# felixchenfy/Monocular-Visual-Odometry

Hardware: AMD Instinct MI355X
Metric: frames/sec (extract+match+5-kf BA), 640x480 / 2000 kp, 1->8 MI355X (higher is better)
Workload: dtype u8 (extract/match) + f64 (BA); 1 GPU

## Files before the change

include/mvo_hip.h:

```cpp
#ifndef MVO_HIP_H
#define MVO_HIP_H
#include <stdint.h>

#ifdef __cplusplus
extern "C" {
#endif

#define MVO_OK 0
#define MVO_ERR_INVALID (-1)
#define MVO_ERR_NO_DEVICE (-2)
#define MVO_ERR_CAPACITY (-3)
#define MVO_ERR_HIP (-4)
#define MVO_ERR_STATE (-5)

typedef struct mvo_ctx mvo_ctx;

typedef struct {
    float x, y, size, angle, response;
    int32_t octave, class_id;
} mvo_keypoint;

typedef struct {
    int32_t queryIdx, trainIdx, imgIdx;
    float distance;
// ... 272 lines not shown
                                  double* angles);
int mvo_rodrigues(const double* rvec, double* R);
int mvo_invert_pose(const double* T, double* T_inv);

int mvo_ba_launch_stats(int device, long long* launches, long long* windows, double* ms, int reset);
int mvo_debug_ba_service_times(int device, double* out5);
int mvo_debug_ba_resident_stats(int device, long long* windows, long long* grid_starts);
int mvo_debug_ba_resident_cycles(int device, double* shader_cycles);
int mvo_debug_ba_path_switches(int device, long long* n);
int mvo_debug_ba_demand_replay(const double* times, int n, uint8_t* decisions);
int mvo_profile_enable(mvo_ctx* ctx, int on);
int mvo_profile_reset(mvo_ctx* ctx);
typedef struct {
    char name[48];
    int64_t launches;
    double total_ms;
} mvo_kernel_time;
int mvo_profile_get(mvo_ctx* ctx, mvo_kernel_time* out, int cap);

int mvo_debug_set(const char* key, int value);
int mvo_debug_ba_trace_enable(mvo_ctx* ctx, int on);
int mvo_debug_get_ba_trace(mvo_ctx* ctx, mvo_ba_handle* handle, double* rows, int cap, int* n);
int mvo_debug_get_ba_plan(mvo_ctx* ctx, mvo_ba_handle* handle, int* wgs, int* nsplit, int32_t* wg_pt_start, int cap);
int mvo_debug_get_ba_phases(mvo_ctx* ctx, long long* cycles, int n, int* wgs);
int mvo_debug_get_level(mvo_ctx* ctx, int level, int blurred, uint8_t* out, int cap, int* w, int* h, int* stride);
int mvo_debug_get_candidates(mvo_ctx* ctx, void* out, int cap, int* n);
int mvo_debug_get_undistort_map(mvo_ctx* ctx, int32_t* ix, int32_t* iy, uint8_t* ax, uint8_t* ay, int cap);

int mvo_debug_get_pnp(mvo_ctx* ctx, double* models, int32_t* counts, int cap, int32_t* info);

int mvo_debug_get_essential(mvo_ctx* ctx, int32_t* counts, int cap_iters, int32_t* info);

int mvo_debug_get_homography(mvo_ctx* ctx, int32_t* counts, int cap_iters, int32_t* info);

int mvo_debug_get_recover_pose(mvo_ctx* ctx, int32_t* good, int32_t* chosen, double* R1R2t, uint8_t* masks, int cap);
int mvo_debug_get_homography_decomposition(mvo_ctx* ctx, double* Hn, double* w, int32_t* branch, double* Rs,
                                           double* ts, double* normals, int32_t* rejected);
int mvo_debug_get_init_finish(mvo_ctx* ctx, float* p_curr, double* cosang, double* pixdist, int cap, int* n);

#ifdef __cplusplus
}
#endif
#endif
```

monocular-visual-odometry_amd/__init__.py:

```python
import ctypes as C
import os

import numpy as np

from . import synth

_HERE = os.path.dirname(os.path.abspath(__file__))
LIB_PATH = os.path.join(_HERE, "csrc", "libmvo_hip.so")
HEADER_PATH = os.path.join(os.path.dirname(_HERE), "include", "mvo_hip.h")

MVO_OK, MVO_ERR_INVALID, MVO_ERR_NO_DEVICE, MVO_ERR_CAPACITY, MVO_ERR_HIP, MVO_ERR_STATE = 0, -1, -2, -3, -4, -5

KEYPOINT_DTYPE = np.dtype([("x", "<f4"), ("y", "<f4"), ("size", "<f4"), ("angle", "<f4"),
                           ("response", "<f4"), ("octave", "<i4"), ("class_id", "<i4")])
DMATCH_DTYPE = np.dtype([("queryIdx", "<i4"), ("trainIdx", "<i4"), ("imgIdx", "<i4"), ("distance", "<f4")])
CANDIDATE_DTYPE = np.dtype([("x", "<i2"), ("y", "<i2"), ("level_score", "<i4"), ("harris", "<f4"), ("angle", "<f4")])
DISTRIBUTE_CANDIDATE_DTYPE = np.dtype([("x", "<i4"), ("y", "<i4"), ("level", "<i4"), ("score", "<i4")])


class OrbParams(C.Structure):
    _fields_ = [("nfeatures", C.c_int32), ("scale_factor", C.c_float), ("nlevels", C.c_int32),
                ("fast_threshold", C.c_int32), ("max_keypoints", C.c_int32), ("grid_size", C.c_int32),
                ("grid_max_per_cell", C.c_int32), ("pyramid_interpolation", C.c_int32)]

# ... 634 lines not shown
        sts = (BaStats * len(problems))()
        self._chk(self.lib.mvo_ba_solve_batch(self.h, prs, len(problems), sts))
        return [(k["poses"].reshape(-1, 4, 4), k["points"], {f: getattr(sts[i], f) for f, _ in BaStats._fields_})
                for i, k in enumerate(keeps)]

    def ba_set_mode(self, mode):
        self._chk(self.lib.mvo_ba_set_mode(self.h, {"latency": 0, "throughput": 1, "shared": 2}[mode]))

    def ba_trace_enable(self, on=True):
        self._chk(self.lib.mvo_debug_ba_trace_enable(self.h, int(on)))

    def ba_trace(self, handle=None, raw_rows=0):
        out = np.zeros((512, 4))
        n = C.c_int()
        self._chk(self.lib.mvo_debug_get_ba_trace(self.h, handle[0] if handle else None, _p(out),
                                                  -int(raw_rows) if raw_rows else 512, C.byref(n)))
        return out[:n.value].copy()

    def ba_plan(self, handle=None):
        g, ns = C.c_int(), C.c_int()
        pt = np.zeros(257, np.int32)
        self._chk(self.lib.mvo_debug_get_ba_plan(self.h, handle[0] if handle else None, C.byref(g), C.byref(ns), _p(pt), 257))
        return dict(wgs=g.value, nsplit=ns.value & 0xffff, groups=max(1, ns.value >> 16), wg_pt_start=pt[:g.value + 1].copy())

    def map_create(self):
        m = C.c_void_p()
        self._chk(self.lib.mvo_map_create(self.h, C.byref(m)))
        return m

    def map_release(self, m):
        self.lib.mvo_map_release.restype = None
        self.lib.mvo_map_release(self.h, m)

    def map_upload(self, m, pos, desc):
        pos = np.ascontiguousarray(pos, np.float32).reshape(-1, 3)
        desc = np.ascontiguousarray(desc, np.uint8).reshape(-1, 32)
        assert len(pos) == len(desc)
        self._chk(self.lib.mvo_map_upload(self.h, m, _p(pos), _p(desc), len(pos)))

    def map_update_positions(self, m, pos, first=0):
        pos = np.ascontiguousarray(pos, np.float32).reshape(-1, 3)
        self._chk(self.lib.mvo_map_update_positions(self.h, m, _p(pos), int(first), len(pos)))

    def map_points_in_view(self, m, T_w_c, K, cols, rows, cap):
        T = np.ascontiguousarray(T_w_c, np.float64).reshape(4, 4)
        idx = np.zeros(max(cap, 1), np.int32)
# ... 445 lines not shown
```

monocular-visual-odometry_amd/csrc/ba_host.cpp:

```cpp
#include <algorithm>
#include <atomic>
#include <cmath>
#include <cstdio>
#include <condition_variable>
#include <cstdlib>
#include <cstring>
#include <chrono>
#include <deque>
#include <map>
#include <mutex>
#include <thread>
#include <vector>

#include "ba_types.h"
#include "mvo_internal.h"

int ba_kernel_set_lds_limit();
hipError_t ba_kernel_launch(const BaBatch& batch, int max_wgs, size_t lds_bytes, hipStream_t stream, int profile, int nr, int slots);
int ba_solver_class(int n);
hipError_t ba_service_launch(const BaServiceArgs& a, hipStream_t stream);

void ba_service_free(int device, void* p, bool host);

int g_ba_use_mfma = 1;
// ... 784 lines not shown
                if (plan_trace)
                    std::fprintf(stderr, "[mvo plan] G %d rows_in_lds %d chunks %d pieces %d pt_passes %d maxEg %d maxLg %d uarea %zu B lds %zu B (budget %d) %s\n",
                                 G, all_lds, nseq, npar, P.npt, maxEg, maxLg, uarea * 8, P.lds, BA_LDS_BUDGET, fits ? "fits" : "-");
                if (all_lds && g_ba_edge_rows != 0) {
                    if (uarea < (size_t)BA_MSTRIDE * (maxEg + 2 * F)) fits = false;
                    break;
                }
            }
        }
        if (fits && maxEg <= BA_EDGE_SLOTS * BA_THREADS && maxLg < 32000) break;
        if (G >= BA_MAX_WGS)
            return mvo_set_err(ctx, MVO_ERR_CAPACITY, "BA window too large for the LDS-resident solver", hipSuccess);
        {
            int next = BA_MAX_WGS;
            for (int c : {2, 4, 8, 16, 32, 64, 128, 256, per_xcd / 2, per_xcd, 2 * per_xcd, 4 * per_xcd, 8 * per_xcd})
                if (c > G && c < next) next = c;
            G = next;
        }
    }
    g_stage_times.lap(0);
    P.nsplit = nsplit;
    P.npar = npar;
    P.nseq = nseq;
    P.uarea = uarea;
    P.G = G;
    P.maxEg = maxEg;
    P.maxLg = maxLg;
    P.groups = 1;
    if (G > 32 && g_ba_groups) {
        int K = 2;
        while (G / K > 32 && K < 8) K *= 2;
        if (G % K == 0 && G / K <= 32 && uarea >= (size_t)K * (size_t)(nlow + nhp)) P.groups = K;
    }
    P.slice = (nlow + G / P.groups - 1) / (G / P.groups);
    std::vector<int>&e_pose = SC.e_pose, &e_point = SC.e_point, &ptstart = SC.ptstart, &ptlist = SC.ptlist;
    std::vector<double>& e_uv = SC.e_uv;
    e_pose.resize(E);
    e_point.resize(E);
    ptstart.assign(L + 1, 0);
    ptlist.resize(E);
    e_uv.resize(2 * (size_t)E);
    {
        std::vector<int>& cur = SC.cur;
        cur.resize((size_t)G * std::max(F, 1));
        for (int g = 0; g < G; ++g)
            for (int q = 0; q < F; ++q) cur[(size_t)g * F + q] = wg_pose[(size_t)g * (F + 1) + q];
        for (int e : act) {
            const int k = cur[(size_t)owner[p->edge_point[e]] * F + p->edge_pose[e]]++;
            e_pose[k] = p->edge_pose[e];
            e_point[k] = p->edge_point[e];
            e_uv[2 * (size_t)k] = p->edge_uv[2 * (size_t)e];
            e_uv[2 * (size_t)k + 1] = p->edge_uv[2 * (size_t)e + 1];
        }
    }
    for (int k = 0; k < E; ++k) ptstart[e_point[k] + 1]++;
// ... 366 lines not shown
    if (H->launched) service_wait(service_for(ctx ? ctx->device : H->ws.device), &H->job, 1);
    ws_free(H->ws);
    delete H;
}

int ba_get_trace(mvo_ctx* ctx, mvo_ba_handle* H, double* rows, int cap, int* n) {
    BaWorkspace* ws = H ? &H->ws : (ctx->ba_pool && !ctx->ba_pool->ws.empty() ? ctx->ba_pool->ws[0] : nullptr);
    if (!ws || !ws->pin) return mvo_set_err(ctx, MVO_ERR_STATE, "no bundle adjustment has run", hipSuccess);
    const BaStatsDev* s = (const BaStatsDev*)(ws->pin + ws->plan.m_stats);
    const int m = cap < 0 ? std::min(-cap, BA_TRACE_MAX) : std::min(std::min(s->trials, BA_TRACE_MAX), cap);
    if (rows) std::memcpy(rows, ws->pin + ws->plan.m_trace, (size_t)m * sizeof(BaTraceRow));
    if (n) *n = m;
    return MVO_OK;
}
int ba_get_plan(mvo_ctx* ctx, mvo_ba_handle* H, int* G, int* nsplit, int32_t* wg_pt, int cap) {
    BaWorkspace* ws = H ? &H->ws : (ctx->ba_pool && !ctx->ba_pool->ws.empty() ? ctx->ba_pool->ws[0] : nullptr);
    if (!ws) return mvo_set_err(ctx, MVO_ERR_STATE, "no bundle adjustment has been planned", hipSuccess);
    if (G) *G = ws->plan.G;
    if (nsplit) *nsplit = ws->plan.nsplit | (ws->plan.groups > 1 ? ws->plan.groups << 16 : 0);
    if (wg_pt)
        for (int i = 0; i <= ws->plan.G && i < cap; ++i) wg_pt[i] = ws->plan.wg_pt[i];
    return MVO_OK;
}
void ba_service_times(int device, double* out5) {
    for (int i = 0; i < 5; ++i) out5[i] = 0;
    if (device < 0 || device >= 16) return;
    BaService* sp;
    {
        std::lock_guard<std::mutex> lk(*g_service_start);
        sp = g_service[device & 15];
    }
    if (!sp) return;
    std::lock_guard<std::mutex> lk(sp->m);
    out5[0] = sp->t_idle, out5[1] = sp->t_batch, out5[2] = sp->t_launch, out5[3] = sp->t_sync, out5[4] = sp->t_post;
}
void ba_service_park(int device) {
    if (device < 0 || device >= 16) return;
    BaService* sp;
    {
        std::lock_guard<std::mutex> lk(*g_service_start);
        sp = g_service[device & 15];
    }
    if (!sp) return;
    std::unique_lock<std::mutex> lk(sp->m);
    if (!sp->resident) return;
    sp->park_requested = true;
// ... 53 lines not shown
```

monocular-visual-odometry_amd/csrc/ba_kernels.hip:

```cpp
#include "ba_types.h"
#include "mvo_internal.h"

typedef ba_u64 u64;
#ifndef MVO_KERNEL_SIM
typedef __attribute__((address_space(1))) double gdouble;
typedef __attribute__((address_space(1))) const u64 gcu64;
typedef __attribute__((address_space(1))) u64 gu64;
#define BA_AS_GLOBAL_D(p) ((gdouble*)(p))
#define BA_AS_GLOBAL_CU64(p) ((gcu64*)(p))
#define BA_AS_GLOBAL_U64(p) ((gu64*)(p))
#else
typedef double gdouble;
typedef const u64 gcu64;
typedef u64 gu64;
#define BA_AS_GLOBAL_D(p) (p)
#define BA_AS_GLOBAL_CU64(p) (p)
#define BA_AS_GLOBAL_U64(p) (p)
#endif

#define PH_BEGIN() long long ph_t = PROF ? (long long)__builtin_amdgcn_s_memtime() : 0
#define PH_END(id)                                                       \
    do {                                                                 \
        if (PROF) {                                                      \
            long long ph_n = (long long)__builtin_amdgcn_s_memtime();    \
// ... 789 lines not shown
    const int msteps = (ncol + 3) / 4;
    const int msplit = (msteps + B.nsplit - 1) / B.nsplit;
    const int chunk_cols = 4 * npar * msplit;
    const short* pkt_g = B.pk_of_tile;
    int pk4[4] = {-1, -1, -1, -1};
    if (do_schur && wave < B.npair * npar) {
#pragma unroll
        for (int j = 0; j < 4; ++j) pk4[j] = pkt_g[(wave % B.npair) * 256 + ((lane >> 4) + 4 * j) * 16 + (lane & 15)];
    }
    EdgeRegs er;
#pragma unroll
    for (int c = 0; c < 6; ++c) er.a0[c] = er.a1[c] = er.x[c] = 0;
    const bool have0 = SLOTS > 0 && tid < Eg, have1 = SLOTS > 1 && tid + BA_THREADS < Eg;
    const int e0_p = have0 ? W.epose[tid] : 0, e0_l = have0 ? W.ept[tid] : 0, e0_sl = have0 ? sSlot[e0_p] : -1;
    constexpr int nslot = SLOTS;
    constexpr int e2_first = SLOTS == 0 ? 0 : BA_THREADS;
#define BA_EDGE_FROM_LDS(BODY, el_)                                          \
    do {                                                                     \
        EdgeRegs r1_;                                                        \
        double ee_[2];                                                       \
        const double* q_ = W.E2 + BA_E2S * ((el_)-e2_first);                 \
        _Pragma("unroll") for (int c_ = 0; c_ < 6; ++c_) {                   \
            r1_.a0[c_] = q_[c_];                                             \
            r1_.a1[c_] = q_[6 + c_];                                         \
            r1_.x[c_] = q_[12 + c_];                                         \
        }                                                                    \
        ee_[0] = q_[18];                                                     \
        ee_[1] = q_[19];                                                     \
        const int p1_ = W.epose[el_];                                        \
        (void)p1_;                                                           \
        BODY(el_, r1_, W.ept[el_], sSlot[p1_], ee_)                          \
    } while (0);
#define BA_EDGES(BODY)                                                       \
    if (nslot > 0 && have0) do { BODY(tid, er, e0_l, e0_sl, ee0) } while (0); \
    if (nslot > 1 && have1) BA_EDGE_FROM_LDS(BODY, tid + BA_THREADS)         \
    if (nslot == 0)                                                          \
        for (int el0_ = tid; el0_ < Eg; el0_ += BA_THREADS) BA_EDGE_FROM_LDS(BODY, el0_)

    int hp_npass = 1;
    {
        const int mcap = (int)(B.uarea / BA_MSTRIDE);
        for (;; ++hp_npass) {
            int tot = 0;
            for (int p = 0; p < B.F; ++p) {
                const int n_p = sPoseStart[p + 1] - sPoseStart[p];
                tot += min(n_p, ((n_p + hp_npass - 1) / hp_npass + 1) & ~1);
            }
            if (tot <= mcap) break;
            if (hp_npass > Eg) {
                error = 1;
                break;
            }
        }
    }
    const bool hp_tables = hp_npass <= BA_HP_PASSES;
    auto hp_slice_row = [&](int q, int row) {
        if (tid < B.F) {
            int off = 0, lo = 0, hi = 0;
            for (int pp = 0; pp <= tid; ++pp) {
                const int s0 = sPoseStart[pp], n_p = sPoseStart[pp + 1] - s0;
                const int h = ((n_p + hp_npass - 1) / hp_npass + 1) & ~1;
                off += hi - lo;
                lo = min(s0 + q * h, s0 + n_p);
                hi = min(s0 + (q + 1) * h, s0 + n_p);
            }
            sSlc[0][row][tid] = (short)lo;
            sSlc[1][row][tid] = (short)hi;
            sSlc[2][row][tid] = (short)off;
        }
    };
    if (hp_tables && !error)
        for (int q = 0; q < hp_npass; ++q) hp_slice_row(q, q);
    int nfp = 0, hp_pa0 = -1, hp_pb0 = -1, hp_pa1 = -1, hp_pb1 = -1;
    for (int p = 0; p < B.F; ++p) {
        if (sSlot[p] < 0) continue;
        if (nfp == 2 * wave) hp_pa0 = p;
        if (nfp == 2 * wave + 1) hp_pb0 = p;
        if (nfp == 2 * (wave + BA_WAVES)) hp_pa1 = p;
        if (nfp == 2 * (wave + BA_WAVES) + 1) hp_pb1 = p;
        ++nfp;
    }
    __syncthreads();

    int piv_hoff = 0;
    if (NR == 32 && n > 0) {
        const int lsh = NR == 32 ? 4 : (n <= 32 ? 4 : (n <= 64 ? 3 : 2)), LPR = 1 << lsh, jj = tid & (LPR - 1);
        const int qi = min(tid >> lsh, n - 1), q0 = min(jj, n - 1), q1 = min(jj + LPR, n - 1);
        piv_hoff = (36 * sSlotPose[qi / 6] + 7 * (qi % 6)) | (36 * sSlotPose[q0 / 6] + 7 * (q0 % 6)) << 10 | (36 * sSlotPose[q1 / 6] + 7 * (q1 % 6)) << 20;
    }
    for (it = 0; any_free && !error && it < B.max_it; ++it) {
        PH_BEGIN();
// ... 10 lines not shown
            const double J0[6] = {x * y / z2 * f, -(1 + (x * x / z2)) * f, y / z * f, -1. / z * f, 0, x / z2 * f};   \
            const double J1[6] = {(1 + y * y / z2) * f, -x * y / z2 * f, -x / z * f, 0, -1. / z * f, y / z2 * f};    \
            _Pragma("unroll") for (int c = 0; c < 6; ++c) {                                                         \
                r.a0[c] = sw * (B.lc00 * J0[c] + B.lc01 * J1[c]);                                                   \
                r.a1[c] = sw * (B.lc11 * J1[c]);                                                                    \
            }                                                                                                       \
        } else {                                                                                                    \
            _Pragma("unroll") for (int c = 0; c < 6; ++c) r.a0[c] = r.a1[c] = 0;                                    \
        }                                                                                                           \
        ee[0] = sw * ew[0];                                                                                         \
        ee[1] = sw * ew[1];                                                                                         \
        _Pragma("unroll") for (int c = 0; c < 6; ++c) r.x[c] = 0;                                                   \
        if (!B.fix_points) {                                                                                        \
            const double* R = sR + 9 * (p);                                                                         \
            const double t0[3] = {f, 0, -x / z * f}, t1[3] = {0, f, -y / z * f};                                    \
            _Pragma("unroll") for (int c = 0; c < 3; ++c) {                                                         \
                double j0 = -1. / z * (t0[0] * R[c] + t0[1] * R[3 + c] + t0[2] * R[6 + c]);                         \
                double j1 = -1. / z * (t1[0] * R[c] + t1[1] * R[3 + c] + t1[2] * R[6 + c]);                         \
                r.x[c] = sw * (B.lc00 * j0 + B.lc01 * j1);                                                          \
                r.x[3 + c] = sw * (B.lc11 * j1);                                                                    \
            }                                                                                                       \
        }                                                                                                           \
    }
        if (nslot > 0 && have0) BA_LINEARIZE(tid, er, e0_p, e0_sl, ee0)
        for (int el = nslot == 0 ? tid : tid + BA_THREADS; nslot != 1 && el < Eg; el += BA_THREADS) {
            EdgeRegs r1;
            double ee[2];
            const int p1 = W.epose[el], sl1 = sSlot[p1];
            BA_LINEARIZE(el, r1, p1, sl1, ee)
            double* q = W.E2 + BA_E2S * (el - e2_first);
#pragma unroll
            for (int c = 0; c < 6; ++c) {
                q[c] = r1.a0[c];
                q[6 + c] = r1.a1[c];
                q[12 + c] = r1.x[c];
            }
            q[18] = ee[0];
            q[19] = ee[1];
        }
        __syncthreads();
        PH_END(0);
        double maxdiag = 0;
        BA_PHASE_HEAD();
        if (!B.fix_points) {
            for (int h = 0; h < B.npt; ++h) {
                const int l_lo = (int)((long long)Lg * h / B.npt), l_hi = (int)((long long)Lg * (h + 1) / B.npt);
                const int k_lo = W.pts0[l_lo], k_hi = W.pts0[l_hi];
#define BA_BODY_STAGE_X(el, r, l_, sl_, ee)                                   \
    const int k_ = W.pti[el];                                                \
    if (k_ < k_lo || k_ >= k_hi) break;                                      \
    double* Xs = stage + BA_SXS * (k_ - k_lo);                               \
    _Pragma("unroll") for (int c = 0; c < 6; ++c) Xs[c] = r.x[c];            \
    Xs[6] = ee[0];                                                           \
    Xs[7] = ee[1];
                BA_EDGES(BA_BODY_STAGE_X)
                __syncthreads();
                for (int l = l_lo + tid; l < l_hi; l += BA_THREADS) {
                    double h6[6] = {0, 0, 0, 0, 0, 0}, b[3] = {0, 0, 0};
                    for (int k = W.pts0[l]; k < W.pts0[l + 1]; ++k) {
                        const double* X = stage + BA_SXS * (k - k_lo);
                        const double e0 = X[6], e1 = X[7];
                        h6[0] += X[0] * X[0] + X[3] * X[3];
                        h6[1] += X[0] * X[1] + X[3] * X[4];
                        h6[2] += X[0] * X[2] + X[3] * X[5];
                        h6[3] += X[1] * X[1] + X[4] * X[4];
                        h6[4] += X[1] * X[2] + X[4] * X[5];
                        h6[5] += X[2] * X[2] + X[5] * X[5];
                        b[0] -= X[0] * e0 + X[3] * e1;
                        b[1] -= X[1] * e0 + X[4] * e1;
                        b[2] -= X[2] * e0 + X[5] * e1;
                    }
#pragma unroll
                    for (int i = 0; i < 6; ++i) W.Hll[BA_XS * l + i] = h6[i];
#pragma unroll
                    for (int i = 0; i < 3; ++i) W.bl[3 * l + i] = b[i];
                    maxdiag = fmax(maxdiag, fmax(fabs(h6[0]), fmax(fabs(h6[3]), fabs(h6[5]))));
                }
                __syncthreads();
            }
        }
        PH_END(2);
        const bool hp_deferred = do_schur && G > 1 && it > 0;
        const bool hp_local = hp_deferred || G == 1;
        if (!hp_deferred) ++tagH;
        BA_PHASE_HEAD();
        {
            const int col = lane & 15;
            v4d accp0 = {0, 0, 0, 0}, accp1 = {0, 0, 0, 0};
            for (int q = 0; q < hp_npass && !error; ++q) {
                const int tq = hp_tables ? q : 0;
                if (!hp_tables) {
                    hp_slice_row(q, 0);
                    __syncthreads();
                }
#define BA_BODY_STAGE_M(el, r, l_, sl_, ee)                                   \
    const int p_ = W.epose[el];                                              \
    const int lo_ = sSlc[0][tq][p_], hi_ = sSlc[1][tq][p_];                  \
    if ((el) < lo_ || (el) >= hi_) break;                                    \
    double* Mr = stage + BA_MSTRIDE * (sSlc[2][tq][p_] + (el)-lo_);          \
    _Pragma("unroll") for (int c = 0; c < 6; ++c) {                          \
        Mr[c] = r.a0[c];                                                     \
        Mr[7 + c] = r.a1[c];                                                 \
    }                                                                        \
    Mr[6] = ee[0];                                                           \
    Mr[13] = ee[1];
                BA_EDGES(BA_BODY_STAGE_M)
                __syncthreads();
                const bool lastq = q == hp_npass - 1;
                if (batch.use_mfma) {
                    int ai = 0;
                    for (int pair = wave; 2 * pair < nfp; pair += BA_WAVES, ++ai) {
                        const int pa = ai == 0 ? hp_pa0 : hp_pa1, pb = ai == 0 ? hp_pb0 : hp_pb1;
                        const bool second = col >= 8;
                        const int pp = second ? pb : pa;
                        const int cc7 = col & 7;
                        const bool cv = cc7 < 7 && pp >= 0;
                        const int rowsA = 2 * (sSlc[1][tq][pa] - sSlc[0][tq][pa]);
                        const int rowsB = pb >= 0 ? 2 * (sSlc[1][tq][pb] - sSlc[0][tq][pb]) : 0;
                        const int s = pp >= 0 ? sSlc[2][tq][pp] : 0, rows = second ? rowsB : rowsA;
                        const int rmax = max(rowsA, rowsB);
                        const double* pm = stage + BA_MSTRIDE * (s + (lane >> 5)) + 7 * ((lane >> 4) & 1) + (cv ? cc7 : 0);
                        const int kq = lane >> 4;
                        const int myrows = cv ? rows - kq : 0;
                        v4d acc = ai == 0 ? accp0 : accp1;
                        int st = 0;
#define BA_HP_LOAD4(V)                                                                   \
    V##0 = 4 * st < myrows ? pm[0] : 0.0, V##1 = 4 * st + 4 < myrows ? pm[2 * BA_MSTRIDE] : 0.0, \
    V##2 = 4 * st + 8 < myrows ? pm[4 * BA_MSTRIDE] : 0.0, V##3 = 4 * st + 12 < myrows ? pm[6 * BA_MSTRIDE] : 0.0; \
    pm += 8 * BA_MSTRIDE;                                                                \
    st += 4
#define BA_HP_MFMA4_LOADNEXT(V, Wn, more)                                      \
    acc = __builtin_amdgcn_mfma_f64_16x16x4f64(V##0, V##0, acc, 0, 0, 0);       \
    __builtin_amdgcn_sched_barrier(0);                                          \
    if (more) { BA_HP_LOAD4(Wn); }                                              \
    __builtin_amdgcn_sched_barrier(0);                                          \
    acc = __builtin_amdgcn_mfma_f64_16x16x4f64(V##1, V##1, acc, 0, 0, 0);       \
    acc = __builtin_amdgcn_mfma_f64_16x16x4f64(V##2, V##2, acc, 0, 0, 0);       \
    acc = __builtin_amdgcn_mfma_f64_16x16x4f64(V##3, V##3, acc, 0, 0, 0)
                        if (4 * (st + 4) <= rmax) {
                            double a0, a1, a2, a3, c0 = 0, c1 = 0, c2 = 0, c3 = 0;
                            BA_HP_LOAD4(a);
                            for (;;) {
                                const bool more1 = 4 * (st + 4) <= rmax;
                                BA_HP_MFMA4_LOADNEXT(a, c, more1);
                                if (!more1) break;
                                const bool more2 = 4 * (st + 4) <= rmax;
                                BA_HP_MFMA4_LOADNEXT(c, a, more2);
                                if (!more2) break;
                            }
                        }
#undef BA_HP_LOAD4
#undef BA_HP_MFMA4_LOADNEXT
                        for (; 4 * st < rmax; ++st) {
                            const double v = 4 * st < myrows ? pm[0] : 0.0;
                            acc = __builtin_amdgcn_mfma_f64_16x16x4f64(v, v, acc, 0, 0, 0);
                            pm += 2 * BA_MSTRIDE;
                        }
                        if (ai == 0) accp0 = acc;
                        else accp1 = acc;
                        if (lastq) {
#pragma unroll
                            for (int j = 0; j < 4; ++j) {
                                const int rg = (lane >> 4) + 4 * j;
                                const bool mine = second ? (rg >= 8 && rg < 15 && pb >= 0) : rg < 7;
                                const int r7 = rg & 7;
                                if (mine && cc7 <= r7 && cc7 < 7) {
                                    const int sl = sSlot[pp], pk = r7 * (r7 + 1) / 2 + cc7;
                                    if (hp_local) W.hpl[BA_HP * sl + pk] = acc[j];
                                    else gstore_d(B.xH + 2 * ((size_t)g * B.nhp + BA_HP * sl + pk), tag0 + tagH, acc[j], same_l2);
                                }
                            }
                        }
                    }
                } else {
                    for (int p = wave; p < B.F; p += BA_WAVES) {
                        const int sl = sSlot[p];
                        if (sl < 0 || lane >= BA_HP) continue;
                        const int lo = sSlc[0][tq][p], hi = sSlc[1][tq][p];
                        const int s = sSlc[2][tq][p], e = s + hi - lo;
                        int i = 0;
                        while ((i + 1) * (i + 2) / 2 <= lane) ++i;
                        const int j = lane - i * (i + 1) / 2;
                        double acc = q == 0 ? 0.0 : W.hpl[BA_HP * sl + lane];
                        for (int r = 2 * s; r < 2 * e; ++r)
                            acc = __builtin_fma(stage[BA_MSTRIDE * (r >> 1) + 7 * (r & 1) + i], stage[BA_MSTRIDE * (r >> 1) + 7 * (r & 1) + j], acc);
                        if (hp_local || !lastq) W.hpl[BA_HP * sl + lane] = acc;
                        else gstore_d(B.xH + 2 * ((size_t)g * B.nhp + BA_HP * sl + lane), tag0 + tagH, acc, same_l2);
                    }
                }
                __syncthreads();
            }
        }
        PH_END(1);
        BA_PHASE_HEAD();
        if (!hp_deferred) {
            const double m = block_max(maxdiag, sScr);
            const int nhp = B.nhp, hrows = min(G, max(1, (int)(B.uarea / nhp)));
            double hsum = 0, mm = 0;
            if (G > 1) {
                if (tid == 0) gstore_d(B.xH + 2 * ((size_t)g * nhp + nhp - 1), tag0 + tagH, m, same_l2);
                for (int w0 = 0; w0 < G; w0 += hrows) {
                    const int nr = min(hrows, G - w0);
                    if (!gather_tagged(B.xH + 2 * (size_t)w0 * nhp, nr * nhp, nhp, nhp, tag0 + tagH, stage)) sFlag[2] = 1;
                    __syncthreads();
                    if (tid < nhp - 1) {
#pragma unroll 8
                        for (int w = 0; w < nr; ++w) hsum += stage[w * nhp + tid];
                    }
                    if (tid < nr) mm = fmax(mm, stage[tid * nhp + nhp - 1]);
                    __syncthreads();
                }
                if (sFlag[2]) error = 1;
            } else {
                if (tid < nhp - 1) hsum = W.hpl[tid];
                if (tid == 0) mm = m;
            }
// ... 736 lines not shown
```

monocular-visual-odometry_amd/csrc/ba_types.h:

```cpp
#ifndef MVO_BA_TYPES_H
#define MVO_BA_TYPES_H
#include <stddef.h>
#include <stdint.h>

typedef unsigned long long ba_u64;

#define BA_THREADS 512
#define BA_WAVES 8
#define BA_MAX_POSES 20
#define BA_MSTRIDE 15
#define BA_XS 7
#define BA_SXS 9
#define BA_EDGE_SLOTS 2
#define BA_PANEL_DOUBLES 1040
#define BA_E2S 21
#define BA_LDS_BUDGET (157 * 1024)
#define BA_MAX_WGS 256
#define BA_MAX_BATCH 16
#define BA_NPHASE 16
#define BA_TRACE_MAX 512
#define BA_HP_PASSES 6
#define BA_HP 28

struct BaStatsDev {
// ... 95 lines not shown
    if (sp > a) a = sp;
    if (sl > a) a = sl;
    return a;
}
__host__ __device__ inline size_t ba_solver_doubles(int n, int nlow, int G, int npair, int npar, int panel, int alias = 0) {
    return (alias ? 0 : ba_solver_matrix_doubles(n, nlow, G, npair, npar)) + 3 * 64 +
           (panel ? BA_PANEL_DOUBLES : 0);
}
__host__ __device__ inline size_t ba_pose_doubles(int F) { return (size_t)(F > 0 ? F : 1) * 82; }
__host__ __device__ inline size_t ba_uarea_doubles(int ucols, int ldu, int max_pt_edges, int maxEpose, int nhp, int G, int fix_points) {
    size_t hrows = 4096 / (size_t)(nhp > 0 ? nhp : 1);
    if (hrows < 1) hrows = 1;
    if (hrows > (size_t)G) hrows = (size_t)G;
    size_t a = (size_t)nhp * hrows;
    const size_t m = (size_t)BA_MSTRIDE * (size_t)(maxEpose > 0 ? maxEpose : 1);
    if (m > a) a = m;
    if (!fix_points) {
        const size_t u = (size_t)ucols * (size_t)(ldu + 1), sx = (size_t)BA_SXS * max_pt_edges;
        if (u > a) a = u;
        if (sx > a) a = sx;
    }
    return a;
}
__host__ __device__ inline size_t ba_lds_bytes(int F, int n, int nlow, int nhp, int G, int npair, int npar, int nfree, int maxEg,
                                               int maxLg, int fix_points, size_t uarea, int e2_edges, int panel, int uv_global = 0,
                                               int alias_sl = 0) {
    size_t d = ba_solver_doubles(n, nlow + nhp, G, npair, npar, panel, alias_sl) + (size_t)nlow + 2 * (size_t)nhp + 17 +
               (uv_global ? 0 : (size_t)maxEg * 2) + (size_t)maxLg * 3;
    d += ba_pose_doubles(F) + 2 * (size_t)G + 8;
    if (!fix_points) d += (size_t)maxLg * (3 + BA_XS + 3 + BA_XS + 3);
    d += uarea + (size_t)e2_edges * BA_E2S;
    size_t shorts = (size_t)maxEg * 5 + (size_t)maxLg + 1 + (size_t)maxLg * (nfree > 0 ? nfree : 1);
    return d * 8 + ((shorts * 2 + 15) & ~(size_t)15) + 64;
}

#endif
```

monocular-visual-odometry_amd/csrc/mvo_api_ba.cpp:

```cpp
#include <cstring>

#include "mvo_internal.h"

int ba_demand_replay(const double* times, int n, unsigned char* decisions);
extern int g_ba_use_mfma, g_ba_wgs, g_ba_same_l2, g_ba_profile, g_ba_block_solver, g_ba_cu_share, g_ba_xcd_reserve, g_ba_edge_rows, g_ba_service, g_ba_chunk_pieces, g_ba_uv_global, g_ba_alias_sl;
int ba_debug_set(const char* key, int value) {
    if (!std::strcmp(key, "ba_mfma")) g_ba_use_mfma = value;
    else if (!std::strcmp(key, "ba_profile")) g_ba_profile = value;
    else if (!std::strcmp(key, "ba_same_l2")) g_ba_same_l2 = value;
    else if (!std::strcmp(key, "ba_wgs")) g_ba_wgs = value;
    else if (!std::strcmp(key, "ba_block_solver")) g_ba_block_solver = value;
    else if (!std::strcmp(key, "ba_cu_share")) g_ba_cu_share = value;
    else if (!std::strcmp(key, "ba_xcd_reserve")) g_ba_xcd_reserve = value;
    else if (!std::strcmp(key, "ba_edge_rows")) g_ba_edge_rows = value;
    else if (!std::strcmp(key, "ba_service")) g_ba_service = value;
    else if (!std::strcmp(key, "ba_chunk_pieces")) g_ba_chunk_pieces = value;
    else if (!std::strcmp(key, "ba_uv_global")) g_ba_uv_global = value;
    else if (!std::strcmp(key, "ba_alias_sl")) g_ba_alias_sl = value;
    else return MVO_ERR_INVALID;
    return MVO_OK;
}

extern "C" {

// ... 88 lines not shown
    if (!shader_cycles) return MVO_ERR_INVALID;
    ba_resident_stats(device, nullptr, nullptr, shader_cycles);
    return MVO_OK;
}

int mvo_ba_launch_stats(int device, long long* launches, long long* windows, double* ms, int reset) {
    if (device < 0 || device > 15) return MVO_ERR_INVALID;
    ba_launch_stats(device, launches, windows, ms, reset);
    return MVO_OK;
}
int mvo_debug_ba_trace_enable(mvo_ctx* ctx, int on) {
    if (!ctx) return MVO_ERR_INVALID;
    ba_set_trace(ctx, on);
    return MVO_OK;
}
int mvo_debug_get_ba_trace(mvo_ctx* ctx, mvo_ba_handle* handle, double* rows, int cap, int* n) {
    if (!ctx) return MVO_ERR_INVALID;
    return ba_get_trace(ctx, handle, rows, cap, n);
}
int mvo_debug_get_ba_plan(mvo_ctx* ctx, mvo_ba_handle* handle, int* wgs, int* nsplit, int32_t* wg_pt_start, int cap) {
    if (!ctx) return MVO_ERR_INVALID;
    return ba_get_plan(ctx, handle, wgs, nsplit, wg_pt_start, cap);
}

int mvo_debug_ba_demand_replay(const double* times, int n, uint8_t* decisions) {
    if (!times || !decisions || n < 0) return MVO_ERR_INVALID;
    return ba_demand_replay(times, n, decisions);
}

int mvo_debug_get_ba_phases(mvo_ctx* ctx, long long* cycles, int n, int* wgs) {
    if (!ctx || !cycles) return MVO_ERR_INVALID;
    for (int i = 0; i < n && i < 16; ++i) cycles[i] = ctx->ba_phase[i];
    if (wgs) *wgs = ctx->ba_wgs;
    return MVO_OK;
}

}
```

monocular-visual-odometry_amd/csrc/mvo_internal.h:

```cpp
#ifndef MVO_INTERNAL_H
#define MVO_INTERNAL_H
#include <hip/hip_runtime.h>
#include <stdint.h>

#ifndef MVO_KERNEL_SIM
#define MVO_DYN_LDS(T, name) extern __shared__ T name[]
#define MVO_DYN_LDS_ALIGNED16(T, name) extern __shared__ __attribute__((aligned(16))) T name[]
#define MVO_WAVES_PER_EU(lo, hi) __attribute__((amdgpu_waves_per_eu(lo, hi)))
#define MVO_WAIT_VM0() asm volatile("s_waitcnt vmcnt(0)" ::: "memory")
#define MVO_OPAQUE(x) asm volatile("" : "+v"(x))
#else
#define MVO_DYN_LDS(T, name) T* name = static_cast<T*>(emu_dyn_lds())
#define MVO_DYN_LDS_ALIGNED16(T, name) T* name = static_cast<T*>(emu_dyn_lds())
#define MVO_WAVES_PER_EU(lo, hi)
#define MVO_WAIT_VM0() __atomic_thread_fence(__ATOMIC_SEQ_CST)
#define MVO_OPAQUE(x) (void)(x)
#endif

#include <algorithm>
#include <chrono>
#include <cstdio>
#include <cstdlib>
#include <map>
#include <atomic>
// ... 497 lines not shown
extern int g_match_mfma;
extern int g_pnp_replay_skew;
void track_release(mvo_ctx* ctx);
struct TrackInitView {
    const float *kp1, *kp2, *pts;
    const int32_t* lists;
    const double *e_out, *h_out;
    uint8_t* out;
};
int track_init_view(mvo_ctx* ctx, int n, int m, TrackInitView* v);
struct mvo_ba_handle;
int ba_solve_device(mvo_ctx* ctx, mvo_ba_problem* p, mvo_ba_stats* st);
int ba_begin_device(mvo_ctx* ctx, const mvo_ba_problem* p);
int ba_end_device(mvo_ctx* ctx, mvo_ba_problem* p, mvo_ba_stats* st);
int ba_solve_batch_device(mvo_ctx* ctx, mvo_ba_problem* ps, int n, mvo_ba_stats* sts);
int ba_prepare_device(mvo_ctx* ctx, const mvo_ba_problem* p, mvo_ba_handle** out);
int ba_run_device(mvo_ctx* ctx, mvo_ba_handle* H);
int ba_fetch_device(mvo_ctx* ctx, mvo_ba_handle* H, double* poses, double* points, mvo_ba_stats* st);
void ba_release_device(mvo_ctx* ctx, mvo_ba_handle* H);
void ba_pool_release(mvo_ctx* ctx);
void ba_set_trace(mvo_ctx* ctx, int on);
int ba_get_trace(mvo_ctx* ctx, mvo_ba_handle* H, double* rows, int cap, int* n);
int ba_get_plan(mvo_ctx* ctx, mvo_ba_handle* H, int* G, int* nsplit, int32_t* wg_pt, int cap);
void ba_launch_stats(int device, long long* launches, long long* windows, double* ms, int reset);
void ba_service_times(int device, double* out5);
void ba_service_park(int device);
void ba_resident_stats(int device, long long* windows, long long* grid_starts, double* cycles = nullptr, long long* path_switches = nullptr);

#endif
```

Measured before the change: 5632 frames/s.

## Build BA pose-block Hessian in place from linearized edge rows

```diff
diff --git a/include/mvo_hip.h b/include/mvo_hip.h
--- a/include/mvo_hip.h
+++ b/include/mvo_hip.h
@@ -318,6 +318,7 @@
 int mvo_debug_ba_trace_enable(mvo_ctx* ctx, int on);
 int mvo_debug_get_ba_trace(mvo_ctx* ctx, mvo_ba_handle* handle, double* rows, int cap, int* n);
 int mvo_debug_get_ba_plan(mvo_ctx* ctx, mvo_ba_handle* handle, int* wgs, int* nsplit, int32_t* wg_pt_start, int cap);
+int mvo_debug_get_ba_layout(mvo_ctx* ctx, mvo_ba_handle* handle, long long* out, int n);
 int mvo_debug_get_ba_phases(mvo_ctx* ctx, long long* cycles, int n, int* wgs);
 int mvo_debug_get_level(mvo_ctx* ctx, int level, int blurred, uint8_t* out, int cap, int* w, int* h, int* stride);
 int mvo_debug_get_candidates(mvo_ctx* ctx, void* out, int cap, int* n);
diff --git a/monocular-visual-odometry_amd/__init__.py b/monocular-visual-odometry_amd/__init__.py
--- a/monocular-visual-odometry_amd/__init__.py
+++ b/monocular-visual-odometry_amd/__init__.py
@@ -680,6 +680,11 @@
         pt = np.zeros(257, np.int32)
         self._chk(self.lib.mvo_debug_get_ba_plan(self.h, handle[0] if handle else None, C.byref(g), C.byref(ns), _p(pt), 257))
         return dict(wgs=g.value, nsplit=ns.value & 0xffff, groups=max(1, ns.value >> 16), wg_pt_start=pt[:g.value + 1].copy())
+
+    def ba_layout(self, handle=None):
+        v = (C.c_longlong * 6)()
+        self._chk(self.lib.mvo_debug_get_ba_layout(self.h, handle[0] if handle else None, v, 6))
+        return dict(zip(("slots", "max_edges", "uarea", "e2_edges", "rows_in_place", "lds_bytes"), (int(x) for x in v)))
 
     def map_create(self):
         m = C.c_void_p()
diff --git a/monocular-visual-odometry_amd/csrc/ba_host.cpp b/monocular-visual-odometry_amd/csrc/ba_host.cpp
--- a/monocular-visual-odometry_amd/csrc/ba_host.cpp
+++ b/monocular-visual-odometry_amd/csrc/ba_host.cpp
@@ -830,6 +830,21 @@
     P.nsplit = nsplit;
     P.npar = npar;
     P.nseq = nseq;
+    const size_t uarea_plan = uarea;
+    {
+        const size_t want = ba_hp_inplace_doubles(P.slots, maxEg);
+        if (want > uarea) {
+            const size_t lds = ba_lds_bytes(F, n, nlow, nhp, G, npair, npar, nfree, maxEg, maxLg, p->fix_points, want, P.e2_edges, P.panel,
+                                            P.uv_global, P.alias_sl);
+            if (lds <= BA_LDS_BUDGET) {
+                uarea = want;
+                P.lds = lds;
+            }
+        }
+        if (plan_trace)
+            std::fprintf(stderr, "[mvo plan] pose-block rows %s: area %zu B (rows in place need %zu B), lds %zu B\n",
+                         uarea >= want ? "in place" : "staged", uarea * 8, want * 8, P.lds);
+    }
     P.uarea = uarea;
     P.G = G;
     P.maxEg = maxEg;
@@ -838,7 +853,7 @@
     if (G > 32 && g_ba_groups) {
         int K = 2;
         while (G / K > 32 && K < 8) K *= 2;
-        if (G % K == 0 && G / K <= 32 && uarea >= (size_t)K * (size_t)(nlow + nhp)) P.groups = K;
+        if (G % K == 0 && G / K <= 32 && uarea_plan >= (size_t)K * (size_t)(nlow + nhp)) P.groups = K;
     }
     P.slice = (nlow + G / P.groups - 1) / (G / P.groups);
     std::vector<int>&e_pose = SC.e_pose, &e_point = SC.e_point, &ptstart = SC.ptstart, &ptlist = SC.ptlist;
@@ -1251,6 +1266,15 @@
         for (int i = 0; i <= ws->plan.G && i < cap; ++i) wg_pt[i] = ws->plan.wg_pt[i];
     return MVO_OK;
 }
+int ba_get_layout(mvo_ctx* ctx, mvo_ba_handle* H, long long* out, int n) {
+    BaWorkspace* ws = H ? &H->ws : (ctx->ba_pool && !ctx->ba_pool->ws.empty() ? ctx->ba_pool->ws[0] : nullptr);
+    if (!ws) return mvo_set_err(ctx, MVO_ERR_STATE, "no bundle adjustment has been planned", hipSuccess);
+    const BaPlan& P = ws->plan;
+    const long long v[6] = {P.slots, P.maxEg, (long long)P.uarea, P.e2_edges,
+                            P.uarea >= ba_hp_inplace_doubles(P.slots, P.maxEg) ? 1 : 0, (long long)P.lds};
+    for (int i = 0; i < n && i < 6; ++i) out[i] = v[i];
+    return MVO_OK;
+}
 void ba_service_times(int device, double* out5) {
     for (int i = 0; i < 5; ++i) out5[i] = 0;
     if (device < 0 || device >= 16) return;
diff --git a/monocular-visual-odometry_amd/csrc/ba_kernels.hip b/monocular-visual-odometry_amd/csrc/ba_kernels.hip
--- a/monocular-visual-odometry_amd/csrc/ba_kernels.hip
+++ b/monocular-visual-odometry_amd/csrc/ba_kernels.hip
@@ -835,11 +835,11 @@
         const double* q_ = W.E2 + BA_E2S * ((el_)-e2_first);                 \
         _Pragma("unroll") for (int c_ = 0; c_ < 6; ++c_) {                   \
             r1_.a0[c_] = q_[c_];                                             \
-            r1_.a1[c_] = q_[6 + c_];                                         \
-            r1_.x[c_] = q_[12 + c_];                                         \
+            r1_.a1[c_] = q_[7 + c_];                                         \
+            r1_.x[c_] = q_[14 + c_];                                         \
         }                                                                    \
-        ee_[0] = q_[18];                                                     \
-        ee_[1] = q_[19];                                                     \
+        ee_[0] = q_[6];                                                      \
+        ee_[1] = q_[13];                                                     \
         const int p1_ = W.epose[el_];                                        \
         (void)p1_;                                                           \
         BODY(el_, r1_, W.ept[el_], sSlot[p1_], ee_)                          \
@@ -850,8 +850,9 @@
     if (nslot == 0)                                                          \
         for (int el0_ = tid; el0_ < Eg; el0_ += BA_THREADS) BA_EDGE_FROM_LDS(BODY, el0_)
 
+    const bool hp_inplace = SLOTS == 0 || (size_t)B.uarea >= ba_hp_inplace_doubles(SLOTS, B.maxEg);
     int hp_npass = 1;
-    {
+    if (!hp_inplace) {
         const int mcap = (int)(B.uarea / BA_MSTRIDE);
         for (;; ++hp_npass) {
             int tot = 0;
@@ -879,7 +880,7 @@
             }
             sSlc[0][row][tid] = (short)lo;
             sSlc[1][row][tid] = (short)hi;
-            sSlc[2][row][tid] = (short)off;
+            sSlc[2][row][tid] = (short)(hp_inplace ? lo : off);
         }
     };
     if (hp_tables && !error)
@@ -936,7 +937,19 @@
             }                                                                                                       \
         }                                                                                                           \
     }
-        if (nslot > 0 && have0) BA_LINEARIZE(tid, er, e0_p, e0_sl, ee0)
+        if (nslot > 0 && have0) {
+            BA_LINEARIZE(tid, er, e0_p, e0_sl, ee0)
+            if (hp_inplace) {
+                double* Mr = stage + (SLOTS == 2 ? B.uarea - BA_MSTRIDE * BA_THREADS : 0) + BA_MSTRIDE * tid;
+#pragma unroll
+                for (int c = 0; c < 6; ++c) {
+                    Mr[c] = er.a0[c];
+                    Mr[7 + c] = er.a1[c];
+                }
+                Mr[6] = ee0[0];
+                Mr[13] = ee0[1];
+            }
+        }
         for (int el = nslot == 0 ? tid : tid + BA_THREADS; nslot != 1 && el < Eg; el += BA_THREADS) {
             EdgeRegs r1;
             double ee[2];
@@ -946,14 +959,157 @@
 #pragma unroll
             for (int c = 0; c < 6; ++c) {
                 q[c] = r1.a0[c];
-                q[6 + c] = r1.a1[c];
-                q[12 + c] = r1.x[c];
-            }
-            q[18] = ee[0];
-            q[19] = ee[1];
+                q[7 + c] = r1.a1[c];
+                q[14 + c] = r1.x[c];
+            }
+            q[6] = ee[0];
+            q[13] = ee[1];
         }
         __syncthreads();
         PH_END(0);
+        const bool hp_deferred = do_schur && G > 1 && it > 0;
+        const bool hp_local = hp_deferred || G == 1;
+        if (!hp_deferred) ++tagH;
+        BA_PHASE_HEAD();
+        {
+            constexpr int HPITCH = SLOTS == 0 ? BA_E2S : BA_MSTRIDE, HPX = BA_E2S - BA_MSTRIDE;
+            const int hp_sw = hp_inplace ? BA_THREADS : 1 << 20;
+            const int hp_base = SLOTS == 0 ? B.uarea : (SLOTS == 2 && hp_inplace ? B.uarea - BA_MSTRIDE * BA_THREADS : 0);
+#define BA_HP_OFF(E) (hp_base + HPITCH * (E) + (SLOTS == 2 ? max(HPX * ((E) - hp_sw), 0) : 0))
+            const int col = lane & 15;
+            v4d accp0 = {0, 0, 0, 0}, accp1 = {0, 0, 0, 0};
+            for (int q = 0; q < hp_npass && !error; ++q) {
+                const int tq = hp_tables ? q : 0;
+                if (!hp_tables) {
+                    hp_slice_row(q, 0);
+                    __syncthreads();
+                }
+#define BA_BODY_STAGE_M(el, r, l_, sl_, ee)                                   \
+    const int p_ = W.epose[el];                                              \
+    const int lo_ = sSlc[0][tq][p_], hi_ = sSlc[1][tq][p_];                  \
+    if ((el) < lo_ || (el) >= hi_) break;                                    \
+    double* Mr = stage + BA_MSTRIDE * (sSlc[2][tq][p_] + (el)-lo_);          \
+    _Pragma("unroll") for (int c = 0; c < 6; ++c) {                          \
+        Mr[c] = r.a0[c];                                                     \
+        Mr[7 + c] = r.a1[c];                                                 \
+    }                                                                        \
+    Mr[6] = ee[0];                                                           \
+    Mr[13] = ee[1];
+                if (!hp_inplace) {
+                    BA_EDGES(BA_BODY_STAGE_M)
+                    __syncthreads();
+                }
+                const bool lastq = q == hp_npass - 1;
+                if (batch.use_mfma) {
+                    int ai = 0;
+                    for (int pair = wave; 2 * pair < nfp; pair += BA_WAVES, ++ai) {
+                        const int pa = ai == 0 ? hp_pa0 : hp_pa1, pb = ai == 0 ? hp_pb0 : hp_pb1;
+                        const bool second = col >= 8;
+                        const int pp = second ? pb : pa;
+                        const int cc7 = col & 7;
+                        const bool cv = cc7 < 7 && pp >= 0;
+                        const int rowsA = 2 * (sSlc[1][tq][pa] - sSlc[0][tq][pa]);
+                        const int rowsB = pb >= 0 ? 2 * (sSlc[1][tq][pb] - sSlc[0][tq][pb]) : 0;
+                        const int s = pp >= 0 ? sSlc[2][tq][pp] : 0, rows = second ? rowsB : rowsA;
+                        const int rmax = __builtin_amdgcn_readfirstlane(max(rowsA, rowsB));
+                        const double* pm = stage + hp_base + 7 * ((lane >> 4) & 1) + (cv ? cc7 : 0);
+                        const int he = s + (lane >> 5);
+                        int rem = cv ? rows / 2 - (lane >> 5) : 0;
+                        int ho = HPITCH * he, h6 = HPX * (he - hp_sw);
+                        v4d acc = ai == 0 ? accp0 : accp1;
+                        int st = 0;
+#define BA_HP_RAW(V, K, R)                                                                         \
+    {                                                                                              \
+        const int i_ = ho + 2 * HPITCH * (K) + (SLOTS == 2 ? max(h6 + 2 * HPX * (K), 0) : 0);      \
+        V = pm[(R) > 2 * (K) ? i_ : 0];                                                            \
+    }
+#define BA_HP_SEL(V, K, R) V = (R) > 2 * (K) ? V : 0.0
+#define BA_HP_ADV(N) ho += 2 * HPITCH * (N), h6 += 2 * HPX * (N)
+#define BA_HP_MFMA4_LOADNEXT(V, Wn, more)                                      \
+    acc = __builtin_amdgcn_mfma_f64_16x16x4f64(V##0, V##0, acc, 0, 0, 0);       \
+    __builtin_amdgcn_sched_barrier(0);                                          \
+    if (more) { BA_HP_RAW(Wn##0, 0, rem - 8) BA_HP_RAW(Wn##1, 1, rem - 8) }     \
+    __builtin_amdgcn_sched_barrier(0);                                          \
+    acc = __builtin_amdgcn_mfma_f64_16x16x4f64(V##1, V##1, acc, 0, 0, 0);       \
+    __builtin_amdgcn_sched_barrier(0);                                          \
+    if (more) {                                                                 \
+        BA_HP_RAW(Wn##2, 2, rem - 8) BA_HP_RAW(Wn##3, 3, rem - 8)               \
+        BA_HP_ADV(4), st += 4;                                                  \
+    }                                                                           \
+    __builtin_amdgcn_sched_barrier(0);                                          \
+    acc = __builtin_amdgcn_mfma_f64_16x16x4f64(V##2, V##2, acc, 0, 0, 0);       \
+    acc = __builtin_amdgcn_mfma_f64_16x16x4f64(V##3, V##3, acc, 0, 0, 0);       \
+    __builtin_amdgcn_sched_barrier(0);                                          \
+    if (more) {                                                                 \
+        rem -= 8;                                                               \
+        BA_HP_SEL(Wn##0, 0, rem), BA_HP_SEL(Wn##1, 1, rem), BA_HP_SEL(Wn##2, 2, rem), BA_HP_SEL(Wn##3, 3, rem); \
+    }                                                                           \
+    __builtin_amdgcn_sched_barrier(0)
+                        if (4 * (st + 4) <= rmax) {
+                            double a0, a1, a2, a3, c0 = 0, c1 = 0, c2 = 0, c3 = 0;
+                            BA_HP_RAW(a0, 0, rem) BA_HP_RAW(a1, 1, rem) BA_HP_RAW(a2, 2, rem) BA_HP_RAW(a3, 3, rem)
+                            BA_HP_ADV(4), st += 4;
+                            BA_HP_SEL(a0, 0, rem), BA_HP_SEL(a1, 1, rem), BA_HP_SEL(a2, 2, rem), BA_HP_SEL(a3, 3, rem);
+                            for (;;) {
+                                const bool more1 = 4 * (st + 4) <= rmax;
+                                BA_HP_MFMA4_LOADNEXT(a, c, more1);
+                                if (!more1) break;
+                                const bool more2 = 4 * (st + 4) <= rmax;
+                                BA_HP_MFMA4_LOADNEXT(c, a, more2);
+                                if (!more2) break;
+                            }
+                            rem -= 8;
+                        }
+#undef BA_HP_MFMA4_LOADNEXT
+                        for (; 4 * st < rmax; ++st) {
+                            double v;
+                            BA_HP_RAW(v, 0, rem)
+                            BA_HP_SEL(v, 0, rem);
+                            acc = __builtin_amdgcn_mfma_f64_16x16x4f64(v, v, acc, 0, 0, 0);
+                            BA_HP_ADV(1), rem -= 2;
+                        }
+#undef BA_HP_RAW
+#undef BA_HP_SEL
+#undef BA_HP_ADV
+                        if (ai == 0) accp0 = acc;
+                        else accp1 = acc;
+                        if (lastq) {
+#pragma unroll
+                            for (int j = 0; j < 4; ++j) {
+                                const int rg = (lane >> 4) + 4 * j;
+                                const bool mine = second ? (rg >= 8 && rg < 15 && pb >= 0) : rg < 7;
+                                const int r7 = rg & 7;
+                                if (mine && cc7 <= r7 && cc7 < 7) {
+                                    const int sl = sSlot[pp], pk = r7 * (r7 + 1) / 2 + cc7;
+                                    if (hp_local) W.hpl[BA_HP * sl + pk] = acc[j];
+                                    else gstore_d(B.xH + 2 * ((size_t)g * B.nhp + BA_HP * sl + pk), tag0 + tagH, acc[j], same_l2);
+                                }
+                            }
+                        }
+                    }
+                } else {
+                    for (int p = wave; p < B.F; p += BA_WAVES) {
+                        const int sl = sSlot[p];
+                        if (sl < 0 || lane >= BA_HP) continue;
+                        const int lo = sSlc[0][tq][p], hi = sSlc[1][tq][p];
+                        const int s = sSlc[2][tq][p], e = s + hi - lo;
+                        int i = 0;
+                        while ((i + 1) * (i + 2) / 2 <= lane) ++i;
+                        const int j = lane - i * (i + 1) / 2;
+                        double acc = q == 0 ? 0.0 : W.hpl[BA_HP * sl + lane];
+                        for (int r = 2 * s; r < 2 * e; ++r) {
+                            const double* row = stage + BA_HP_OFF(r >> 1) + 7 * (r & 1);
+                            acc = __builtin_fma(row[i], row[j], acc);
+                        }
+                        if (hp_local || !lastq) W.hpl[BA_HP * sl + lane] = acc;
+                        else gstore_d(B.xH + 2 * ((size_t)g * B.nhp + BA_HP * sl + lane), tag0 + tagH, acc, same_l2);
+                    }
+                }
+                __syncthreads();
+            }
+#undef BA_HP_OFF
+        }
+        PH_END(1);
         double maxdiag = 0;
         BA_PHASE_HEAD();
         if (!B.fix_points) {
@@ -994,118 +1150,6 @@
             }
         }
         PH_END(2);
-        const bool hp_deferred = do_schur && G > 1 && it > 0;
-        const bool hp_local = hp_deferred || G == 1;
-        if (!hp_deferred) ++tagH;
-        BA_PHASE_HEAD();
-        {
-            const int col = lane & 15;
-            v4d accp0 = {0, 0, 0, 0}, accp1 = {0, 0, 0, 0};
-            for (int q = 0; q < hp_npass && !error; ++q) {
-                const int tq = hp_tables ? q : 0;
-                if (!hp_tables) {
-                    hp_slice_row(q, 0);
-                    __syncthreads();
-                }
-#define BA_BODY_STAGE_M(el, r, l_, sl_, ee)                                   \
-    const int p_ = W.epose[el];                                              \
-    const int lo_ = sSlc[0][tq][p_], hi_ = sSlc[1][tq][p_];                  \
-    if ((el) < lo_ || (el) >= hi_) break;                                    \
-    double* Mr = stage + BA_MSTRIDE * (sSlc[2][tq][p_] + (el)-lo_);          \
-    _Pragma("unroll") for (int c = 0; c < 6; ++c) {                          \
-        Mr[c] = r.a0[c];                                                     \
-        Mr[7 + c] = r.a1[c];                                                 \
-    }                                                                        \
-    Mr[6] = ee[0];                                                           \
-    Mr[13] = ee[1];
-                BA_EDGES(BA_BODY_STAGE_M)
-                __syncthreads();
-                const bool lastq = q == hp_npass - 1;
-                if (batch.use_mfma) {
-                    int ai = 0;
-                    for (int pair = wave; 2 * pair < nfp; pair += BA_WAVES, ++ai) {
-                        const int pa = ai == 0 ? hp_pa0 : hp_pa1, pb = ai == 0 ? hp_pb0 : hp_pb1;
-                        const bool second = col >= 8;
-                        const int pp = second ? pb : pa;
-                        const int cc7 = col & 7;
-                        const bool cv = cc7 < 7 && pp >= 0;
-                        const int rowsA = 2 * (sSlc[1][tq][pa] - sSlc[0][tq][pa]);
-                        const int rowsB = pb >= 0 ? 2 * (sSlc[1][tq][pb] - sSlc[0][tq][pb]) : 0;
-                        const int s = pp >= 0 ? sSlc[2][tq][pp] : 0, rows = second ? rowsB : rowsA;
-                        const int rmax = max(rowsA, rowsB);
-                        const double* pm = stage + BA_MSTRIDE * (s + (lane >> 5)) + 7 * ((lane >> 4) & 1) + (cv ? cc7 : 0);
-                        const int kq = lane >> 4;
-                        const int myrows = cv ? rows - kq : 0;
-                        v4d acc = ai == 0 ? accp0 : accp1;
-                        int st = 0;
-#define BA_HP_LOAD4(V)                                                                   \
-    V##0 = 4 * st < myrows ? pm[0] : 0.0, V##1 = 4 * st + 4 < myrows ? pm[2 * BA_MSTRIDE] : 0.0, \
-    V##2 = 4 * st + 8 < myrows ? pm[4 * BA_MSTRIDE] : 0.0, V##3 = 4 * st + 12 < myrows ? pm[6 * BA_MSTRIDE] : 0.0; \
-    pm += 8 * BA_MSTRIDE;                                                                \
-    st += 4
-#define BA_HP_MFMA4_LOADNEXT(V, Wn, more)                                      \
-    acc = __builtin_amdgcn_mfma_f64_16x16x4f64(V##0, V##0, acc, 0, 0, 0);       \
-    __builtin_amdgcn_sched_barrier(0);                                          \
-    if (more) { BA_HP_LOAD4(Wn); }                                              \
-    __builtin_amdgcn_sched_barrier(0);                                          \
-    acc = __builtin_amdgcn_mfma_f64_16x16x4f64(V##1, V##1, acc, 0, 0, 0);       \
-    acc = __builtin_amdgcn_mfma_f64_16x16x4f64(V##2, V##2, acc, 0, 0, 0);       \
-    acc = __builtin_amdgcn_mfma_f64_16x16x4f64(V##3, V##3, acc, 0, 0, 0)
-                        if (4 * (st + 4) <= rmax) {
-                            double a0, a1, a2, a3, c0 = 0, c1 = 0, c2 = 0, c3 = 0;
-                            BA_HP_LOAD4(a);
-                            for (;;) {
-                                const bool more1 = 4 * (st + 4) <= rmax;
-                                BA_HP_MFMA4_LOADNEXT(a, c, more1);
-                                if (!more1) break;
-                                const bool more2 = 4 * (st + 4) <= rmax;
-                                BA_HP_MFMA4_LOADNEXT(c, a, more2);
-                                if (!more2) break;
-                            }
-                        }
-#undef BA_HP_LOAD4
-#undef BA_HP_MFMA4_LOADNEXT
-                        for (; 4 * st < rmax; ++st) {
-                            const double v = 4 * st < myrows ? pm[0] : 0.0;
-                            acc = __builtin_amdgcn_mfma_f64_16x16x4f64(v, v, acc, 0, 0, 0);
-                            pm += 2 * BA_MSTRIDE;
-                        }
-                        if (ai == 0) accp0 = acc;
-                        else accp1 = acc;
-                        if (lastq) {
-#pragma unroll
-                            for (int j = 0; j < 4; ++j) {
-                                const int rg = (lane >> 4) + 4 * j;
-                                const bool mine = second ? (rg >= 8 && rg < 15 && pb >= 0) : rg < 7;
-                                const int r7 = rg & 7;
-                                if (mine && cc7 <= r7 && cc7 < 7) {
-                                    const int sl = sSlot[pp], pk = r7 * (r7 + 1) / 2 + cc7;
-                                    if (hp_local) W.hpl[BA_HP * sl + pk] = acc[j];
-                                    else gstore_d(B.xH + 2 * ((size_t)g * B.nhp + BA_HP * sl + pk), tag0 + tagH, acc[j], same_l2);
-                                }
-                            }
-                        }
-                    }
-                } else {
-                    for (int p = wave; p < B.F; p += BA_WAVES) {
-                        const int sl = sSlot[p];
-                        if (sl < 0 || lane >= BA_HP) continue;
-                        const int lo = sSlc[0][tq][p], hi = sSlc[1][tq][p];
-                        const int s = sSlc[2][tq][p], e = s + hi - lo;
-                        int i = 0;
-                        while ((i + 1) * (i + 2) / 2 <= lane) ++i;
-                        const int j = lane - i * (i + 1) / 2;
-                        double acc = q == 0 ? 0.0 : W.hpl[BA_HP * sl + lane];
-                        for (int r = 2 * s; r < 2 * e; ++r)
-                            acc = __builtin_fma(stage[BA_MSTRIDE * (r >> 1) + 7 * (r & 1) + i], stage[BA_MSTRIDE * (r >> 1) + 7 * (r & 1) + j], acc);
-                        if (hp_local || !lastq) W.hpl[BA_HP * sl + lane] = acc;
-                        else gstore_d(B.xH + 2 * ((size_t)g * B.nhp + BA_HP * sl + lane), tag0 + tagH, acc, same_l2);
-                    }
-                }
-                __syncthreads();
-            }
-        }
-        PH_END(1);
         BA_PHASE_HEAD();
         if (!hp_deferred) {
             const double m = block_max(maxdiag, sScr);
diff --git a/monocular-visual-odometry_amd/csrc/ba_types.h b/monocular-visual-odometry_amd/csrc/ba_types.h
--- a/monocular-visual-odometry_amd/csrc/ba_types.h
+++ b/monocular-visual-odometry_amd/csrc/ba_types.h
@@ -141,6 +141,9 @@
     }
     return a;
 }
+__host__ __device__ inline size_t ba_hp_inplace_doubles(int slots, int maxEg) {
+    return slots == 0 ? 0 : (size_t)BA_MSTRIDE * (size_t)(maxEg < BA_THREADS ? maxEg : BA_THREADS);
+}
 __host__ __device__ inline size_t ba_lds_bytes(int F, int n, int nlow, int nhp, int G, int npair, int npar, int nfree, int maxEg,
                                                int maxLg, int fix_points, size_t uarea, int e2_edges, int panel, int uv_global = 0,
                                                int alias_sl = 0) {
diff --git a/monocular-visual-odometry_amd/csrc/mvo_api_ba.cpp b/monocular-visual-odometry_amd/csrc/mvo_api_ba.cpp
--- a/monocular-visual-odometry_amd/csrc/mvo_api_ba.cpp
+++ b/monocular-visual-odometry_amd/csrc/mvo_api_ba.cpp
@@ -134,6 +134,10 @@
     if (!ctx) return MVO_ERR_INVALID;
     return ba_get_plan(ctx, handle, wgs, nsplit, wg_pt_start, cap);
 }
+int mvo_debug_get_ba_layout(mvo_ctx* ctx, mvo_ba_handle* handle, long long* out, int n) {
+    if (!ctx || !out) return MVO_ERR_INVALID;
+    return ba_get_layout(ctx, handle, out, n);
+}
 
 int mvo_debug_ba_demand_replay(const double* times, int n, uint8_t* decisions) {
     if (!times || !decisions || n < 0) return MVO_ERR_INVALID;
diff --git a/monocular-visual-odometry_amd/csrc/mvo_internal.h b/monocular-visual-odometry_amd/csrc/mvo_internal.h
--- a/monocular-visual-odometry_amd/csrc/mvo_internal.h
+++ b/monocular-visual-odometry_amd/csrc/mvo_internal.h
@@ -543,6 +543,7 @@
 void ba_set_trace(mvo_ctx* ctx, int on);
 int ba_get_trace(mvo_ctx* ctx, mvo_ba_handle* H, double* rows, int cap, int* n);
 int ba_get_plan(mvo_ctx* ctx, mvo_ba_handle* H, int* G, int* nsplit, int32_t* wg_pt, int cap);
+int ba_get_layout(mvo_ctx* ctx, mvo_ba_handle* H, long long* out, int n);
 void ba_launch_stats(int device, long long* launches, long long* windows, double* ms, int reset);
 void ba_service_times(int device, double* out5);
 void ba_service_park(int device);
```

Result: faster. 5696 frames/s (median of 6 runs) (+1.1%).
